# facebookresearch/dmc-net

Hardware: AMD Instinct MI355X
Metric: clips/sec (3-seg 224x224) DMC-gen+ResNet-18 train step (higher is better)
Workload: dtype f32

## Files before the change

### dmc-net_amd/csrc/conv_x3s.hip

```cpp
#include "dmc_common.h"
#include "x3s_common.h"
#include <type_traits>

using namespace dmc;
using namespace dmc::x3;

namespace {

__global__ __launch_bounds__(256) void x3s_split_kernel(const float* __restrict__ x, unsigned short* __restrict__ xs, long M, int C) {
    const int c8 = C >> 3;
    const long total = M * c8;
    const int nchunk = C >> 4;
    for (long o = (long)blockIdx.x * 256 + threadIdx.x; o < total; o += (long)gridDim.x * 256) {
        const long m = o / c8;
        const int g = (int)(o - m * c8);
        const float4 a = reinterpret_cast<const float4*>(x)[2 * o], b = reinterpret_cast<const float4*>(x)[2 * o + 1];
        const float v[8] = {a.x, a.y, a.z, a.w, b.x, b.y, b.z, b.w};
        x3s_store8(xs, v, (size_t)M, nchunk, (size_t)m, g);
    }
}

__global__ __launch_bounds__(256) void x3s_merge_kernel(const unsigned short* __restrict__ xs, float* __restrict__ x, long M, int C) {
    const long total = M * C;
    const size_t plane = (size_t)M * 16;
    const int nchunk = C >> 4;
    for (long o = (long)blockIdx.x * 256 + threadIdx.x; o < total; o += (long)gridDim.x * 256) {
        const long m = o / C;
        const int c = (int)(o - m * C);
        const size_t w = ((size_t)(c >> 4) * M + m) * 16 + (c & 15);
        const float a = __uint_as_float((unsigned)xs[w] << 16);
        const float b = __uint_as_float((unsigned)xs[(size_t)nchunk * plane + w] << 16);
        const float d = __uint_as_float((unsigned)xs[(size_t)2 * nchunk * plane + w] << 16);
        x[o] = (a + b) + d;
    }
}

__global__ __launch_bounds__(256) void x3s_pack_w_kernel(const float* __restrict__ w, unsigned short* __restrict__ wf,
                                                         unsigned short* __restrict__ wt, int Cout, int Cin, int mirror) {
    const bool transposed = blockIdx.y == 1;
    unsigned short* dst = transposed ? wt : wf;
    if (!dst) return;
    const int R = transposed ? Cin : Cout, K = transposed ? Cout : Cin;
    const int nchunk = K >> 4;
    const long total = (long)R * 9 * K;
    for (long i = (long)blockIdx.x * 256 + threadIdx.x; i < total; i += (long)gridDim.x * 256) {
        long t = i;
        const int kk = (int)(t & 15); t >>= 4;
        const int rl = (int)(t & 63); t >>= 6;
        const int tap = (int)(t % 9); t /= 9;
        const int ch = (int)(t % nchunk);
        const int rt = (int)(t / nchunk);
        const int r = rt * 64 + rl, k = ch * 16 + kk;
        const float v = transposed ? w[((long)k * 9 + (mirror ? 8 - tap : tap)) * Cin + r] : w[((long)r * 9 + tap) * Cin + k];
        unsigned s0, s1, s2;
        split3_bf16(v, s0, s1, s2);
        const size_t base = ((((size_t)(rt * nchunk + ch) * 9 + tap) * 3) * 64 + rl) * 16 + (kk ^ (((rl >> 3) & 1) << 3));
        dst[base] = (unsigned short)s0;
        dst[base + 64 * 16] = (unsigned short)s1;
        dst[base + 2 * 64 * 16] = (unsigned short)s2;
    }
}

struct X3Args {
    const void* xs;
    const void* wp;
    float* y;
    const float* addend;
    double* stat_part;
    int N, H, W, K, R;
    int M;
    unsigned plane_bytes;
    const float* bnb_y = nullptr;
    const float* bnb_stats = nullptr;
    const float* bnb_gamma = nullptr;
    const float* bnb_beta = nullptr;
    const unsigned char* bnb_mask = nullptr;
    int bnb_relu = 0;
    double* bnb_part = nullptr;
    int part_blocks = -1;
    int ablate;
};
struct X3EvalArgs : X3Args {
    const float* stats;
    const float* gamma;
    const float* beta;
    const float* res;
    unsigned short* ys;
    int s2d, relu;
};

template <int WM, int WN, int TM, int TN, int PPMAX, bool STAG = false, int CLS = 1, bool EVAL = false>
__global__ __launch_bounds__(WM * WN * 64) void x3s_conv_kernel(std::conditional_t<EVAL, X3EvalArgs, X3Args> a) {
    static_assert(!EVAL || CLS == 1, "the eval epilogue belongs to the forward convolution");
    constexpr int NW = WM * WN, BM = 32 * TM * WM, BN = 32 * TN * WN;
    static_assert(BN == 64, "packed weight image is 64 rows wide");
    static_assert(PPMAX % 32 == 0 || PPMAX % 32 == 1, "patch transfers move 32 pixel rows");
    constexpr int PSL = PPMAX * 32;
    constexpr int PB = 3 * PSL;
    constexpr int WB = 3 * 3 * BN * 32;
    constexpr int WOFF = 2 * PB;
    static_assert(!STAG || NW >= 4, "two transfer groups need four waves");
    constexpr int NA = STAG ? NW / 2 : NW, NB = NW - (STAG ? NA : 0);
    constexpr int NDW = (PPMAX / 32 + NA - 1) / NA;
    constexpr int NEW = WB / 1024;
    constexpr int NEWW = (NEW + NB - 1) / NB;
    extern __shared__ __attribute__((aligned(1024))) char lds_x3[];

    const int tid = threadIdx.x, lane = tid & 63;
    const int wave = __builtin_amdgcn_readfirstlane(tid >> 6);
    const int wm = wave % WM, wn = wave / WM;
    const int l31 = lane & 31, khalf = lane >> 5;
    const unsigned lds0 = lds_addr_of(lds_x3);

    const int HW = a.H * a.W, PW = a.W;
    constexpr int ZROW = PPMAX - 1;
    const int m0 = blockIdx.x * BM;
    const int mlast = (m0 + BM < a.M ? m0 + BM : a.M) - 1;
    const int r_first = m0 / PW, r_last = mlast / PW;
    const int f0 = (r_first > 0 ? r_first - 1 : 0) * PW;
    const int f1 = (r_last + 2) * PW < a.M ? (r_last + 2) * PW : a.M;
    const int PP = f1 - f0;
    const int ND = (PP + 31) >> 5;

    unsigned pvoff[NDW];
#pragma unroll
    for (int k = 0; k < NDW; ++k) {
        const int pr = 32 * (wave + NA * k) + (lane >> 1), h = lane & 1;
        pvoff[k] = pr < PP ? (unsigned)(f0 + pr) * 32u + (unsigned)((h ^ ((pr >> 3) & 1)) << 4) : OOB;
    }
    int xaddr[TM][9];
#pragma unroll
    for (int i = 0; i < TM; ++i) {
        int m = m0 + (wm * TM + i) * 32 + l31;
        if (m > mlast) m = mlast;
        const int n = m / HW, rem = m - n * HW, yy = rem / a.W, xx = rem - yy * a.W;
        const int pp = m - f0;
#pragma unroll
        for (int t = 0; t < 9; ++t) {
            const int dx = CLS == 4 ? (t % 3 == 0 ? 1 : 0) : t % 3 - 1, dy = CLS == 4 ? (t / 3 == 0 ? 1 : 0) : t / 3 - 1;
            const int row = (xx + dx >= 0 && xx + dx < a.W && yy + dy >= 0 && yy + dy < a.H) ? pp + dy * PW + dx : ZROW;
            xaddr[i][t] = row * 32 + ((khalf ^ ((row >> 3) & 1)) << 4);
        }
    }
    const int waddr = (wn * TN * 32 + l31) * 32 + ((khalf ^ ((l31 >> 3) & 1)) << 4);

    const u32x4 srd_x = make_srd(a.xs);
    const int nchunk = a.K >> 4, S = 3 * nchunk;
    const u32x4 srd_w = make_srd(reinterpret_cast<const char*>(a.wp) + (size_t)blockIdx.y * S * WB);
    const unsigned lane16 = (unsigned)lane * 16u;

    const bool grp_a = wave < NA, grp_b = !STAG || wave >= NA;
    const int wb = STAG ? wave - NA : wave;
    auto dma_weight = [&](int step, int wbuf, int k) {
        const int e = wb + NB * k;
        if (e < NEW) dma_buf16(srd_w, lane16, (unsigned)(step * WB + e * 1024), lds0 + WOFF + wbuf * WB + e * 1024);
    };
    auto dma_patch = [&](int chunk, int slice, int pbuf, int k) {
        const int d = wave + NA * k;
        if (d < ND) dma_buf16(srd_x, pvoff[k], (unsigned)(slice * nchunk + chunk) * a.plane_bytes, lds0 + pbuf * PB + slice * PSL + d * 1024);
    };
    auto issue_weights = [&](int step, int wbuf) {
        if (grp_b) {
#pragma unroll
            for (int k = 0; k < NEWW; ++k) dma_weight(step, wbuf, k);
        }
    };
    auto issue_patch = [&](int chunk, int slice, int pbuf) {
        if (grp_a) {
#pragma unroll
            for (int k = 0; k < NDW; ++k) dma_patch(chunk, slice, pbuf, k);
        }
    };

    f32x16 acc[CLS][TM][TN];
#pragma unroll
    for (int cl = 0; cl < CLS; ++cl)
#pragma unroll
        for (int i = 0; i < TM; ++i)
#pragma unroll
            for (int j = 0; j < TN; ++j)
#pragma unroll
                for (int e = 0; e < 16; ++e) acc[cl][i][j][e] = 0.f;

    lds_cptr const L = (lds_cptr)lds_x3;
    struct Frag { u32x4 X[TM][3], W[TN][3]; };
    auto load_frags = [&](auto pbufc, auto wbufc, auto tc, Frag& f) {
        constexpr int pbuf = decltype(pbufc)::value, wbuf = decltype(wbufc)::value, t = decltype(tc)::value;
#pragma unroll
        for (int s = 0; s < 3; ++s) {
#pragma unroll
            for (int j = 0; j < TN; ++j)
                f.W[j][s] = *reinterpret_cast<const __attribute__((address_space(3))) u32x4*>(
                    L + waddr + (WOFF + wbuf * WB + (((t % 3) * 3 + s) * BN + 32 * j) * 32));
#pragma unroll
            for (int i = 0; i < TM; ++i)
                f.X[i][s] = *reinterpret_cast<const __attribute__((address_space(3))) u32x4*>(L + xaddr[i][t] + (pbuf * PB + s * PSL));
        }
    };
    auto mfma_frags = [&](const Frag& f, auto tc, auto&& between) {
        constexpr int t = decltype(tc)::value;
        constexpr int cl = CLS == 4 ? (t / 3 != 1) * 2 + (t % 3 != 1) : 0;
#pragma unroll
        for (int p = 0; p < 6; ++p) {
            constexpr int WS[6] = {0, 0, 0, 1, 1, 2}, XS[6] = {2, 1, 0, 1, 0, 0};
#pragma unroll
            for (int i = 0; i < TM; ++i)
#pragma unroll
                for (int j = 0; j < TN; ++j) acc[cl][i][j] = mfma_bf16(f.W[j][WS[p]], f.X[i][XS[p]], acc[cl][i][j]);
            between(p);
        }
    };
    auto nothing = [](int) {};
    constexpr int NRD = 3 * (TM + TN), NMF = 6 * TM * TN;
    auto interleave = [&]() {
#pragma unroll
        for (int k = 0; k < NRD; ++k) {
            __builtin_amdgcn_sched_group_barrier(0x008, 1, 0);
            __builtin_amdgcn_sched_group_barrier(0x100, 1, 0);
        }
        __builtin_amdgcn_sched_group_barrier(0x008, NMF - NRD, 0);
    };
    const bool dma_on = !(DMC_ABL(a.ablate) & 64);
    auto step = [&](auto pbufc, auto wbufc, auto qc, Frag& FA, Frag& FB, int c) {
        constexpr int pbuf = decltype(pbufc)::value, wbuf = decltype(wbufc)::value, q = decltype(qc)::value;
        using NP = std::integral_constant<int, q == 2 ? (pbuf ^ 1) : pbuf>;
        using NWB = std::integral_constant<int, wbuf ^ 1>;
        using NT = std::integral_constant<int, q == 2 ? 0 : 3 * (q + 1)>;
        using T0 = std::integral_constant<int, 3 * q>;
        using T1 = std::integral_constant<int, 3 * q + 1>;
        using T2 = std::integral_constant<int, 3 * q + 2>;
        const int s = 3 * c + q;
        load_frags(pbufc, wbufc, std::integral_constant<int, 3 * q + 1>{}, FB);
        if constexpr (STAG) {
            const bool go = grp_b && dma_on && s + 1 < S;
            mfma_frags(FA, T0{}, [&](int p) {
                if (go) {
#pragma unroll
                    for (int k = p; k < NEWW; k += 6) dma_weight(s + 1, wbuf ^ 1, k);
                }
            });
        } else {
            mfma_frags(FA, T0{}, nothing);
            interleave();
        }
        load_frags(pbufc, wbufc, std::integral_constant<int, 3 * q + 2>{}, FA);
        mfma_frags(FB, T1{}, nothing);
        interleave();
        if (DMC_ABL(a.ablate) & 16) asm volatile("s_waitcnt lgkmcnt(0)" ::: "memory");
        else asm volatile("s_waitcnt vmcnt(0) lgkmcnt(0)" ::: "memory");
        __builtin_amdgcn_s_barrier();
        const int vc = q == 2 ? c + 2 : c + 1;
        if constexpr (STAG) {
            if (s + 1 < S) load_frags(NP{}, NWB{}, NT{}, FB);
            const bool go = grp_a && dma_on && vc < nchunk;
            mfma_frags(FA, T2{}, [&](int p) {
                if (go) {
#pragma unroll
                    for (int k = p; k < NDW; k += 6) dma_patch(vc, q == 2 ? 0 : q + 1, q == 2 ? pbuf : (pbuf ^ 1), k);
                }
            });
        } else {
            if (dma_on) {
                if (s + 2 < S) issue_weights(s + 2, wbuf);
                if (vc < nchunk) issue_patch(vc, q == 2 ? 0 : q + 1, q == 2 ? pbuf : (pbuf ^ 1));
            }
            if (s + 1 < S) load_frags(NP{}, NWB{}, NT{}, FB);
            mfma_frags(FA, T2{}, nothing);
        }
    };
    using I0 = std::integral_constant<int, 0>;
    using I1 = std::integral_constant<int, 1>;
    using Q0 = std::integral_constant<int, 0>;
    using Q1 = std::integral_constant<int, 1>;
    using Q2 = std::integral_constant<int, 2>;

    if (tid < 12)
        *reinterpret_cast<float4*>(lds_x3 + (tid >> 1) * PSL + ZROW * 32 + (tid & 1) * 16) = make_float4(0.f, 0.f, 0.f, 0.f);
    issue_weights(0, 0);
    issue_patch(0, 0, 0); issue_patch(0, 1, 0); issue_patch(0, 2, 0);
    asm volatile("s_waitcnt vmcnt(0)" ::: "memory");
    __builtin_amdgcn_s_barrier();
    if (dma_on) {
        if (!STAG && S > 1) issue_weights(1, 1);
        if (nchunk > 1) issue_patch(1, 0, 1);
    }
    Frag F0, F1;
    load_frags(I0{}, I0{}, Q0{}, F0);
#pragma unroll 1
    for (int c = 0; c < ((DMC_ABL(a.ablate) & 256) ? 0 : nchunk); c += 2) {
        step(I0{}, I0{}, Q0{}, F0, F1, c);
        step(I0{}, I1{}, Q1{}, F1, F0, c);
        step(I0{}, I0{}, Q2{}, F0, F1, c);
        step(I1{}, I1{}, Q0{}, F1, F0, c + 1);
        step(I1{}, I0{}, Q1{}, F0, F1, c + 1);
        step(I1{}, I1{}, Q2{}, F1, F0, c + 1);
    }

    static_assert(WN == 1 && TN == 2, "epilogue: a wave owns all 64 channels of its pixels");
    constexpr int EP = 272, ETILE = 32 * TM * EP;
    char* etile = lds_x3 + wave * ETILE;
    const int mw0 = m0 + wm * TM * 32;
    const int rbase = blockIdx.y * BN;
#pragma unroll
    for (int cl = 0; cl < CLS; ++cl) {
#pragma unroll
        for (int i = 0; i < TM; ++i) {
            const bool ok = mw0 + 32 * i + l31 <= mlast;
#pragma unroll
            for (int j = 0; j < TN; ++j)
#pragma unroll
                for (int g = 0; g < 4; ++g) {
                    float4 v = make_float4(acc[cl][i][j][4 * g], acc[cl][i][j][4 * g + 1], acc[cl][i][j][4 * g + 2], acc[cl][i][j][4 * g + 3]);
                    if (!ok) v = make_float4(0.f, 0.f, 0.f, 0.f);
                    *reinterpret_cast<float4*>(etile + (32 * i + l31) * EP + (32 * j + 8 * g + 4 * khalf) * 4) = v;
                }
        }
        if constexpr (EVAL) {
            const int c4 = rbase + (lane & 15) * 4;
            const float4 mean = *reinterpret_cast<const float4*>(a.stats + c4), istd = *reinterpret_cast<const float4*>(a.stats + a.R + c4);
            const float4 gm = *reinterpret_cast<const float4*>(a.gamma + c4), bt = *reinterpret_cast<const float4*>(a.beta + c4);
            const bool has_res = a.res != nullptr, relu = a.relu != 0;
            const int ochunk = a.R >> 4;
#pragma unroll
            for (int it = 0; it < 8 * TM; ++it) {
                const int prow = 4 * it + (lane >> 4);
                const int m = mw0 + prow;
                const float4 v = *reinterpret_cast<const float4*>(etile + prow * EP + (lane & 15) * 16);
                if (m <= mlast) {
                    const size_t o = (size_t)m * a.R + c4;
                    float4 rv = make_float4(0.f, 0.f, 0.f, 0.f);
                    if (has_res) rv = *reinterpret_cast<const float4*>(a.res + o);
                    const float w[4] = {bn_apply_act1(v.x, mean.x, istd.x, gm.x, bt.x, has_res, rv.x, relu),
                                        bn_apply_act1(v.y, mean.y, istd.y, gm.y, bt.y, has_res, rv.y, relu),
                                        bn_apply_act1(v.z, mean.z, istd.z, gm.z, bt.z, has_res, rv.z, relu),
                                        bn_apply_act1(v.w, mean.w, istd.w, gm.w, bt.w, has_res, rv.w, relu)};
                    if (a.y) *reinterpret_cast<float4*>(a.y + o) = make_float4(w[0], w[1], w[2], w[3]);
                    if (a.ys) {
                        if (a.s2d) {
                            const int n = m / HW, rem = m - n * HW, yy = rem / a.W, xx = rem - yy * a.W;
                            const int cls = (yy & 1) * 2 + (xx & 1);
                            const size_t mq = ((size_t)n * (a.H >> 1) + (yy >> 1)) * (a.W >> 1) + (xx >> 1);
                            x3s_store4(a.ys, w, (size_t)a.M >> 2, 4 * ochunk, mq, (c4 >> 2) + cls * 4 * ochunk);
                        } else {
                            x3s_store4(a.ys, w, (size_t)a.M, ochunk, (size_t)m, c4 >> 2);
                        }
                    }
                }
            }
        } else
        if (!(DMC_ABL(a.ablate) & 128)) {
#pragma unroll
            for (int it = 0; it < 8 * TM; ++it) {
                const int prow = 4 * it + (lane >> 4);
                const int m = mw0 + prow;
                float4 v = *reinterpret_cast<const float4*>(etile + prow * EP + (lane & 15) * 16);
                if (m <= mlast) {
                    size_t opix = (size_t)m;
                    if (CLS == 4) {
                        const int n = m / HW, rem = m - n * HW, ya = rem / a.W, xb = rem - ya * a.W;
                        opix = ((size_t)n * (2 * a.H) + 2 * ya + (cl >> 1)) * (2 * a.W) + 2 * xb + (cl & 1);
                    }
                    const size_t o = opix * a.R + rbase + (lane & 15) * 4;
                    if (a.addend) {
                        const float4 av = *reinterpret_cast<const float4*>(a.addend + o);
                        v.x += av.x; v.y += av.y; v.z += av.z; v.w += av.w;
                    }
                    *reinterpret_cast<float4*>(a.y + o) = v;
                    if (CLS == 1 && a.bnb_part) {
                        const int c4 = rbase + (lane & 15) * 4;
                        const float4 yv = *reinterpret_cast<const float4*>(a.bnb_y + o);
                        const float4 mean = *reinterpret_cast<const float4*>(a.bnb_stats + c4);
                        const float4 istd = *reinterpret_cast<const float4*>(a.bnb_stats + a.R + c4);
                        const float4 xh = make_float4((yv.x - mean.x) * istd.x, (yv.y - mean.y) * istd.y, (yv.z - mean.z) * istd.z, (yv.w - mean.w) * istd.w);
                        if (a.bnb_relu) {
                            unsigned mb;
                            if (a.bnb_mask) {
                                mb = a.bnb_mask[o >> 2];
                            } else {
                                const float4 g = *reinterpret_cast<const float4*>(a.bnb_gamma + c4), b = *reinterpret_cast<const float4*>(a.bnb_beta + c4);
                                mb = (fmaf(xh.x, g.x, b.x) > 0.f ? 1u : 0u) | (fmaf(xh.y, g.y, b.y) > 0.f ? 2u : 0u) |
                                     (fmaf(xh.z, g.z, b.z) > 0.f ? 4u : 0u) | (fmaf(xh.w, g.w, b.w) > 0.f ? 8u : 0u);
                            }
                            v.x = (mb & 1) ? v.x : 0.f; v.y = (mb & 2) ? v.y : 0.f; v.z = (mb & 4) ? v.z : 0.f; v.w = (mb & 8) ? v.w : 0.f;
                        }
                        *reinterpret_cast<float4*>(etile + prow * EP + (lane & 15) * 16) = v;
                        *reinterpret_cast<float4*>(etile + NW * ETILE + 8192 + prow * EP + (lane & 15) * 16) = xh;
                    }
                } else if (CLS == 1 && a.bnb_part) {
                    *reinterpret_cast<float4*>(etile + prow * EP + (lane & 15) * 16) = make_float4(0.f, 0.f, 0.f, 0.f);
                    *reinterpret_cast<float4*>(etile + NW * ETILE + 8192 + prow * EP + (lane & 15) * 16) = make_float4(0.f, 0.f, 0.f, 0.f);
                }
            }
        }
    }
    if constexpr (EVAL) return;
    if (CLS == 1 && a.bnb_part) {
        double* red = reinterpret_cast<double*>(lds_x3 + NW * ETILE);
        const char* xtile = etile + NW * ETILE + 8192;
        double d1 = 0.0, d2 = 0.0;
#pragma unroll 8
        for (int p = 0; p < 32 * TM; ++p) {
            const double d = (double)*reinterpret_cast<const float*>(etile + p * EP + lane * 4);
            const double xh = (double)*reinterpret_cast<const float*>(xtile + p * EP + lane * 4);
            d1 += d;
            d2 += d * xh;
        }
        red[(wm * 64 + lane) * 2 + 0] = d1;
        red[(wm * 64 + lane) * 2 + 1] = d2;
        __syncthreads();
        for (int cc = tid; cc < BN; cc += NW * 64) {
            double e1 = 0.0, e2 = 0.0;
#pragma unroll
            for (int w = 0; w < WM; ++w) { e1 += red[(w * 64 + cc) * 2 + 0]; e2 += red[(w * 64 + cc) * 2 + 1]; }
            double* dst = a.bnb_part + ((size_t)blockIdx.x * a.R + rbase + cc) * 2;
            dst[0] = e1; dst[1] = e2;
        }
    }
    if (CLS == 1 && a.stat_part) {
        double* red = reinterpret_cast<double*>(lds_x3 + NW * ETILE);
        double d1 = 0.0, d2 = 0.0;
#pragma unroll 8
        for (int p = 0; p < 32 * TM; ++p) {
            const double v = (double)*reinterpret_cast<const float*>(etile + p * EP + lane * 4);
            d1 += v;
            d2 += v * v;
        }
        red[(wm * 64 + lane) * 2 + 0] = d1;
        red[(wm * 64 + lane) * 2 + 1] = d2;
        __syncthreads();
        for (int c = tid; c < BN; c += NW * 64) {
            double e1 = 0.0, e2 = 0.0;
#pragma unroll
            for (int w = 0; w < WM; ++w) { e1 += red[(w * 64 + c) * 2 + 0]; e2 += red[(w * 64 + c) * 2 + 1]; }
            double* dst = a.stat_part + ((size_t)blockIdx.x * a.R + rbase + c) * 2;
            dst[0] = e1; dst[1] = e2;
        }
    }
}

int patch_pixels_max(int N, int H, int W, int BM) {
    const long M = (long)N * H * W;
    int worst = 0;
    long tiles = (M + BM - 1) / BM;
    if (tiles > W) tiles = W;
    for (long t = 0; t < tiles; ++t) {
        const long m0 = t * BM, ml = (m0 + BM < M ? m0 + BM : M) - 1;
        const long r0 = m0 / W, r1 = ml / W;
        const long f0 = (r0 > 0 ? r0 - 1 : 0) * W, f1 = (r1 + 2) * W;
        if ((int)(f1 - f0) + 1 > worst) worst = (int)(f1 - f0) + 1;
    }
    return worst;
}

struct X3Cfg { int id, BM, PPMAX, threads; };
constexpr X3Cfg X3CFGS[] = {{0, 256, 608, 512}, {1, 128, 320, 256}, {2, 64, 192, 128}, {3, 256, 608, 256}, {4, 128, 225, 256}};

bool x3s_shape_ok(int N, int H, int W, int K, int R) {
    if (N <= 0 || H <= 0 || W <= 0 || K % 32 != 0 || R % 64 != 0 || K <= 0 || R <= 0) return false;
    const long M = (long)N * H * W;
    return M * (K > R ? K : R) * 6 < (1L << 31);
}

int x3s_choose(int N, int H, int W, int R) {
    const long M = (long)N * H * W;
    const int forced = option(OPT_CONV_CFG);
    if (forced >= 101 && forced <= 105 && patch_pixels_max(N, H, W, X3CFGS[forced - 101].BM) <= X3CFGS[forced - 101].PPMAX) return forced - 101;
    if (forced != 106 && patch_pixels_max(N, H, W, X3CFGS[4].BM) <= X3CFGS[4].PPMAX && ((M + X3CFGS[4].BM - 1) / X3CFGS[4].BM) * (R / 64) >= 512)
        return 4;
    int fallback = -1;
    for (const X3Cfg& c : X3CFGS) {
        if (c.id > 2 || patch_pixels_max(N, H, W, c.BM) > c.PPMAX) continue;
        const long wgs = ((M + c.BM - 1) / c.BM) * (R / 64);
        if (wgs >= 160) return c.id;
        fallback = c.id;
    }
    return fallback;
}

template <int WM, int TM, int PPMAX>
int launch_x3s(const X3Args& a, hipStream_t s) {
    constexpr int BM = 32 * TM * WM;
    constexpr size_t op_bytes = 2 * 3 * PPMAX * 32 + 2 * 3 * 3 * 64 * 32, ep_bytes = 2 * (size_t)BM * 272 + 8192;
    constexpr size_t lds_bytes = op_bytes > ep_bytes ? op_bytes : ep_bytes;
    dim3 grid((a.M + BM - 1) / BM, a.R / 64);
    if ((a.stat_part || a.bnb_part) && a.part_blocks >= 0 && (unsigned)a.part_blocks != grid.x)
        return fail(DMC_E_INVALID, "x3s_conv: statistics partials have %d rows but this launch writes %u (dmc_x3s_conv_stat_blocks was "
                                   "called under another conv_cfg option?)", a.part_blocks, grid.x);
    if constexpr (WM >= 4) {
        if (!(option(OPT_CONV_ABLATE) & 512)) {
            static LdsLimit lim_attr2;
    const hipError_t attr2 = lim_attr2.raise(reinterpret_cast<const void*>(&x3s_conv_kernel<WM, 1, TM, 2, PPMAX, true>), (int)lds_bytes);
            if (attr2 != hipSuccess) return fail(DMC_E_LAUNCH, "x3s_conv: cannot raise the dynamic LDS limit: %s", hipGetErrorString(attr2));
            x3s_conv_kernel<WM, 1, TM, 2, PPMAX, true><<<grid, WM * 64, lds_bytes, s>>>(a);
            return check_launch("x3s_conv");
        }
    }
    static LdsLimit lim_attr;
    const hipError_t attr = lim_attr.raise(reinterpret_cast<const void*>(&x3s_conv_kernel<WM, 1, TM, 2, PPMAX>), (int)lds_bytes);
    if (attr != hipSuccess) return fail(DMC_E_LAUNCH, "x3s_conv: cannot raise the dynamic LDS limit: %s", hipGetErrorString(attr));
    x3s_conv_kernel<WM, 1, TM, 2, PPMAX><<<grid, WM * 64, lds_bytes, s>>>(a);
    return check_launch("x3s_conv");
}

struct X3Bnb { const float *y, *stats, *gamma, *beta; const unsigned char* mask; int relu; double* part; };

int run_x3s(const void* xs, const void* wp, const float* addend, float* y, double* stat_part, int part_blocks, int N, int H, int W,
            int K, int R, hipStream_t s, const X3Bnb* bnb = nullptr) {
    if (!xs || !wp || !y) return fail(DMC_E_INVALID, "x3s_conv: null pointer");
    if (!x3s_shape_ok(N, H, W, K, R)) return fail(DMC_E_INVALID, "x3s_conv: unsupported shape N=%d H=%d W=%d K=%d R=%d", N, H, W, K, R);
    const int cfg = x3s_choose(N, H, W, R);
    X3Args a;
    a.xs = xs; a.wp = wp; a.y = y; a.addend = addend; a.stat_part = stat_part;
    a.N = N; a.H = H; a.W = W; a.K = K; a.R = R; a.M = N * H * W;
    a.plane_bytes = (unsigned)a.M * 32u;
    a.part_blocks = part_blocks;
    if ((stat_part || bnb) && part_blocks <= 0) return fail(DMC_E_INVALID, "x3s_conv: stat_blocks must be the row count of the partials");
    if (bnb) {
        a.bnb_y = bnb->y; a.bnb_stats = bnb->stats; a.bnb_gamma = bnb->gamma; a.bnb_beta = bnb->beta; a.bnb_mask = bnb->mask;
        a.bnb_relu = bnb->relu; a.bnb_part = bnb->part;
    }
    a.ablate = option(OPT_CONV_ABLATE);
    if (DMC_ABL(a.ablate) & 32) a.stat_part = nullptr;
    switch (cfg) {
        case 0: return launch_x3s<8, 1, 608>(a, s);
        case 1: return launch_x3s<4, 1, 320>(a, s);
        case 2: return launch_x3s<2, 1, 192>(a, s);
        case 3: return launch_x3s<4, 2, 608>(a, s);
        case 4: return launch_x3s<4, 1, 225>(a, s);
        default: return fail(DMC_E_INVALID, "x3s_conv: the patch of a %d x %d image does not fit the LDS", H, W);
    }
}

template <int WM, int TM, int PPMAX>
int launch_x3s_eval(const X3EvalArgs& a, hipStream_t s) {
    constexpr int BM = 32 * TM * WM;
    constexpr size_t lds_bytes = 2 * 3 * PPMAX * 32 + 2 * 3 * 3 * 64 * 32;
    static_assert((size_t)BM * 272 <= lds_bytes, "the epilogue tiles live in the operand LDS");
    dim3 grid((a.M + BM - 1) / BM, a.R / 64);
    static LdsLimit lim_attr;
    const hipError_t attr = lim_attr.raise(reinterpret_cast<const void*>(&x3s_conv_kernel<WM, 1, TM, 2, PPMAX, (WM >= 4), 1, true>), (int)lds_bytes);
    if (attr != hipSuccess) return fail(DMC_E_LAUNCH, "x3s_conv_bn_eval: cannot raise the dynamic LDS limit: %s", hipGetErrorString(attr));
    x3s_conv_kernel<WM, 1, TM, 2, PPMAX, (WM >= 4), 1, true><<<grid, WM * 64, lds_bytes, s>>>(a);
    return check_launch("x3s_conv_bn_eval");
}

struct X3WgArgs {
    const void* xs;
    const void* dys;
    float* part;
    int N, H, Cin, Cout;
    unsigned plane_bytes;
    int steps, per_group, tiles_ci;
};

template <int W_, int R>
struct WgGeom {
    static constexpr int PW = W_ + 2;
    static constexpr int NGRP = R >= W_ + 2 ? 2 : 4, LA = NGRP / 2;
    static constexpr int NRING = NGRP * R;
    static constexpr int XPX = NRING * PW;
    static constexpr int XPL = ((XPX + 3) / 8) * 8 + 4;
    static constexpr int NPX = R * W_;
    static constexpr int NKB = (NPX + 15) / 16;
    static constexpr int DYP = NKB * 16;
    static constexpr int DYT = ((DYP + 31) / 32) * 32;
    static constexpr int DYPL = ((DYT + 3) / 8) * 8 + 4;
    static constexpr int XI = (R * PW + 31) / 32;
    static constexpr int DI = DYT / 32;
    static constexpr int XBYTES = 12 * XPL * 32, DYBYTES = 12 * DYPL * 32;
    static constexpr int LDS = XBYTES + 2 * DYBYTES;
};

template <int W_, int R>
__global__ __launch_bounds__(768) void x3s_wgrad_kernel(X3WgArgs a) {
    using G = WgGeom<W_, R>;
    constexpr int PW = G::PW, NRING = G::NRING, XPL = G::XPL, DYPL = G::DYPL, NKB = G::NKB;
    extern __shared__ __attribute__((aligned(1024))) char lds_wg[];
    const int tid = threadIdx.x, lane = tid & 63;
    const int wave = __builtin_amdgcn_readfirstlane(tid >> 6);
    const int l31 = lane & 31, khalf = lane >> 5, L = lane & 15, grp = (lane >> 4) & 1;
    const int quarter = wave & 3, trow = wave >> 2;
    const int wi = quarter & 1, wj = quarter >> 1;
    const int tci = blockIdx.x % a.tiles_ci, tco = blockIdx.x / a.tiles_ci;
    const unsigned lds0 = lds_addr_of(lds_wg);
    const int HP = a.H + 2;
    const int s_begin = blockIdx.y * a.per_group;
    const int s_end = s_begin + a.per_group < a.steps ? s_begin + a.per_group : a.steps;
    const u32x4 srd_x = make_srd(a.xs), srd_d = make_srd(a.dys);
    const unsigned soff_x = (unsigned)((wave >> 2) * (a.Cin >> 4) + tci * 4 + (wave & 3)) * a.plane_bytes;
    const unsigned soff_d = (unsigned)((wave >> 2) * (a.Cout >> 4) + tco * 4 + (wave & 3)) * a.plane_bytes;
    const unsigned xplane = lds0 + (unsigned)wave * XPL * 32, dplane = lds0 + G::XBYTES + (unsigned)wave * DYPL * 32;
    const int lpx = lane >> 1;
    const unsigned lhalf = (unsigned)(lane & 1) << 4;

    const unsigned img_bytes = (unsigned)(a.H * W_) * 32u;
    unsigned xpre[G::XI], dpre[G::DI];
#pragma unroll
    for (int i = 0; i < G::XI; ++i) {
        const int px = 32 * i + lpx;
        const int r = px / PW, col = px - r * PW - 1;
        xpre[i] = (col >= 0 && col < W_) ? (unsigned)(r * W_ + col) * 32u + lhalf : NOPIX;
    }
#pragma unroll
    for (int i = 0; i < G::DI; ++i) {
        const int p = 32 * i + lpx;
        dpre[i] = p < G::NPX ? (unsigned)p * 32u + lhalf : NOPIX;
    }
    auto issue_x = [&](int q, const WgGroupPos& g) {
        const int slot0 = (((q % G::NGRP) + G::NGRP) % G::NGRP) * R;
        unsigned tbase, img_off;
        wg_group_base(g, a.N, W_, img_bytes, tbase, img_off);
#pragma unroll
        for (int i = 0; i < G::XI; ++i)
            if (32 * i + lpx < R * PW)
                dma_buf16(srd_x, wg_lane_off(tbase, xpre[i], img_bytes), soff_x + img_off, xplane + (unsigned)(slot0 * PW + 32 * i) * 32u);
    };
    auto issue_dy = [&](const WgGroupPos& g, int buf) {
        unsigned tbase, img_off;
        wg_group_base(g, a.N, W_, img_bytes, tbase, img_off);
#pragma unroll
        for (int i = 0; i < G::DI; ++i)
            dma_buf16(srd_d, wg_lane_off(tbase, dpre[i], img_bytes), soff_d + img_off, dplane + (unsigned)buf * G::DYBYTES + (unsigned)(32 * i) * 32u);
    };

    f32x16 acc[3];
// ... 89 lines not shown
    p.per_group = (p.steps + groups - 1) / groups;
    p.groups = (p.steps + p.per_group - 1) / p.per_group;
    return true;
}

template <int W_, int R>
int launch_x3s_wgrad(const X3WgPlan& p, X3WgArgs a, float* dw, hipStream_t s) {
    using G = WgGeom<W_, R>;
    static_assert(G::LDS <= 160 * 1024, "weight-gradient tiles exceed the LDS");
    static LdsLimit lim_attr;
    const hipError_t attr = lim_attr.raise(reinterpret_cast<const void*>(&x3s_wgrad_kernel<W_, R>), G::LDS);
    if (attr != hipSuccess) return fail(DMC_E_LAUNCH, "x3s_wgrad: cannot raise the dynamic LDS limit: %s", hipGetErrorString(attr));
    x3s_wgrad_kernel<W_, R><<<dim3(p.tiles, p.groups), 768, G::LDS, s>>>(a);
    int rc = check_launch("x3s_wgrad");
    if (rc || p.groups == 1) return rc;
    const long numel = (long)a.Cout * 9 * a.Cin;
    const long blocks = (numel + 63) / 64;
    x3s_wgrad_reduce_kernel<<<(int)(blocks > 4096 ? 4096 : blocks), 256, 0, s>>>(a.part, dw, p.groups, numel);
    return check_launch("x3s_wgrad_reduce");
}

__global__ __launch_bounds__(256) void x3s_bnb_final_kernel(const double* __restrict__ part, int nblk, int C,
                                                            float* __restrict__ dgamma, float* __restrict__ dbeta) {
    __shared__ double red[2][4];
    const int c = blockIdx.x, lane = threadIdx.x & 63, wave = threadIdx.x >> 6;
    double s = 0.0, ss = 0.0;
    for (int b = threadIdx.x; b < nblk; b += 256) {
        const double2 v = *reinterpret_cast<const double2*>(part + ((size_t)b * C + c) * 2);
        s += v.x;
        ss += v.y;
    }
#pragma unroll
    for (int o = 32; o > 0; o >>= 1) { s += __shfl_down(s, o, 64); ss += __shfl_down(ss, o, 64); }
    if (lane == 0) { red[0][wave] = s; red[1][wave] = ss; }
    __syncthreads();
    if (threadIdx.x != 0) return;
    dbeta[c] = (float)(red[0][0] + red[0][1] + red[0][2] + red[0][3]);
    dgamma[c] = (float)(red[1][0] + red[1][1] + red[1][2] + red[1][3]);
}

int stream_blocks(long total) {
    long b = (total + 255) / 256;
    return (int)(b < 1 ? 1 : (b > 8192 ? 8192 : b));
}

}

extern "C" {

size_t dmc_x3s_slices_bytes(long M, int C) { return (size_t)M * (size_t)C * 6; }

int dmc_x3s_split(const float* x, void* xs, long M, int C, dmc_stream_t stream) {
    if (!x || !xs || M <= 0 || C <= 0 || C % 16 != 0) return fail(DMC_E_INVALID, "dmc_x3s_split: bad argument");
    x3s_split_kernel<<<stream_blocks(M * (C / 8)), 256, 0, (hipStream_t)stream>>>(x, static_cast<unsigned short*>(xs), M, C);
    return check_launch("x3s_split");
}

int dmc_x3s_merge(const void* xs, float* x, long M, int C, dmc_stream_t stream) {
    if (!x || !xs || M <= 0 || C <= 0 || C % 16 != 0) return fail(DMC_E_INVALID, "dmc_x3s_merge: bad argument");
    x3s_merge_kernel<<<stream_blocks(M * C), 256, 0, (hipStream_t)stream>>>(static_cast<const unsigned short*>(xs), x, M, C);
    return check_launch("x3s_merge");
}

size_t dmc_x3s_wpack_bytes(int Cin, int Cout) { return (size_t)Cin * (size_t)Cout * 9 * 6; }

int dmc_x3s_pack_weights(const float* w, void* wpack_f, void* wpack_t, int Cin, int Cout, dmc_stream_t stream) {
    if (!w || (!wpack_f && !wpack_t) || Cin % 64 != 0 || Cout % 64 != 0 || Cin <= 0 || Cout <= 0)
        return fail(DMC_E_INVALID, "dmc_x3s_pack_weights: bad argument");
    const long total = (long)Cin * Cout * 9;
    x3s_pack_w_kernel<<<dim3(stream_blocks(total) > 1024 ? 1024 : stream_blocks(total), 2), 256, 0, (hipStream_t)stream>>>(
        w, static_cast<unsigned short*>(wpack_f), static_cast<unsigned short*>(wpack_t), Cout, Cin, 1);
    return check_launch("x3s_pack_w");
}

int dmc_x3s_conv_supported(int N, int H, int W, int Cin, int Cout) {
    return Cin % 64 == 0 && Cout % 64 == 0 && x3s_shape_ok(N, H, W, Cin, Cout) && x3s_shape_ok(N, H, W, Cout, Cin) &&
           x3s_choose(N, H, W, Cout) >= 0 && x3s_choose(N, H, W, Cin) >= 0 ? 1 : 0;
}

int dmc_x3s_conv_stat_blocks(int N, int H, int W, int Cout) {
    const int cfg = x3s_choose(N, H, W, Cout);
    if (cfg < 0) return 0;
    const long M = (long)N * H * W;
    return (int)((M + X3CFGS[cfg].BM - 1) / X3CFGS[cfg].BM);
}

int dmc_x3s_conv_fwd(const void* xs, const void* wpack_f, float* y, double* stat_partials, int stat_blocks, int N, int H, int W,
                     int Cin, int Cout, dmc_stream_t stream) {
    return run_x3s(xs, wpack_f, nullptr, y, stat_partials, stat_blocks, N, H, W, Cin, Cout, (hipStream_t)stream);
}

int dmc_x3s_conv_bn_eval(const void* xs, const void* wpack_f, const float* stats, const float* gamma, const float* beta,
                         const float* residual, float* y, void* ys, int s2d, int relu, int N, int H, int W, int Cin, int Cout,
                         dmc_stream_t stream) {
    if (!xs || !wpack_f || !stats || !gamma || !beta) return fail(DMC_E_INVALID, "dmc_x3s_conv_bn_eval: null pointer");
    if (!y && !ys) return fail(DMC_E_INVALID, "dmc_x3s_conv_bn_eval: no output (y and ys are both null)");
    if (s2d && !ys) return fail(DMC_E_INVALID, "dmc_x3s_conv_bn_eval: s2d describes the slice output, which is null");
    if (s2d && ((H & 1) || (W & 1))) return fail(DMC_E_INVALID, "dmc_x3s_conv_bn_eval: a space-to-depth result needs even H and W (H=%d W=%d)", H, W);
    if (Cin % 64 != 0 || Cout % 64 != 0 || !x3s_shape_ok(N, H, W, Cin, Cout) || !x3s_shape_ok(N, H, W, Cout, Cin))
        return fail(DMC_E_INVALID, "dmc_x3s_conv_bn_eval: unsupported shape N=%d H=%d W=%d Cin=%d Cout=%d", N, H, W, Cin, Cout);
    X3EvalArgs a;
    a.xs = xs; a.wp = wpack_f; a.y = y; a.addend = nullptr; a.stat_part = nullptr;
    a.N = N; a.H = H; a.W = W; a.K = Cin; a.R = Cout; a.M = N * H * W;
    a.plane_bytes = (unsigned)a.M * 32u;
    a.ablate = 0;
    a.stats = stats; a.gamma = gamma; a.beta = beta; a.res = residual; a.ys = static_cast<unsigned short*>(ys);
    a.s2d = s2d ? 1 : 0; a.relu = relu ? 1 : 0;
    hipStream_t s = (hipStream_t)stream;
    switch (x3s_choose(N, H, W, Cout)) {
        case 0: return launch_x3s_eval<8, 1, 608>(a, s);
        case 1: return launch_x3s_eval<4, 1, 320>(a, s);
        case 2: return launch_x3s_eval<2, 1, 192>(a, s);
        case 3: return launch_x3s_eval<4, 2, 608>(a, s);
        case 4: return launch_x3s_eval<4, 1, 225>(a, s);
        default: return fail(DMC_E_INVALID, "dmc_x3s_conv_bn_eval: the patch of a %d x %d image does not fit the LDS", H, W);
    }
}

int dmc_x3s_conv_dgrad(const void* dys, const void* wpack_t, const float* addend, float* dx, int N, int H, int W, int Cin, int Cout,
                       dmc_stream_t stream) {
    return run_x3s(dys, wpack_t, addend, dx, nullptr, -1, N, H, W, Cout, Cin, (hipStream_t)stream);
}

int dmc_x3s_conv_wgrad_supported(int N, int H, int W, int Cin, int Cout) {
    X3WgPlan p;
    return x3s_wgrad_plan(N, H, W, Cin, Cout, p) && x3s_shape_ok(N, H, W, Cin, Cout) && x3s_shape_ok(N, H, W, Cout, Cin) ? 1 : 0;
}

size_t dmc_x3s_conv_wgrad_bytes(int N, int H, int W, int Cin, int Cout) {
    X3WgPlan p;
    if (!x3s_wgrad_plan(N, H, W, Cin, Cout, p) || p.groups <= 1) return 0;
    return (size_t)p.groups * Cout * 9 * Cin * sizeof(float);
}

int dmc_x3s_conv_wgrad(const void* xs, const void* dys, float* dw, float* workspace, int N, int H, int W, int Cin, int Cout,
                       dmc_stream_t stream) {
    X3WgPlan p;
    if (!xs || !dys || !dw) return fail(DMC_E_INVALID, "dmc_x3s_conv_wgrad: null pointer");
    if (!dmc_x3s_conv_wgrad_supported(N, H, W, Cin, Cout) || !x3s_wgrad_plan(N, H, W, Cin, Cout, p))
        return fail(DMC_E_INVALID, "dmc_x3s_conv_wgrad: unsupported shape N=%d H=%d W=%d Cin=%d Cout=%d", N, H, W, Cin, Cout);
    if (p.groups > 1 && !workspace) return fail(DMC_E_INVALID, "dmc_x3s_conv_wgrad: workspace required");
    X3WgArgs a;
    a.xs = xs; a.dys = dys; a.part = p.groups > 1 ? workspace : dw;
    a.N = N; a.H = H; a.Cin = Cin; a.Cout = Cout;
    a.plane_bytes = (unsigned)((long)N * H * W) * 32u;
    a.steps = p.steps; a.per_group = p.per_group; a.tiles_ci = Cin / 64;
    hipStream_t s = (hipStream_t)stream;
    switch (W) {
        case 56: return launch_x3s_wgrad<56, 1>(p, a, dw, s);
        case 28: return launch_x3s_wgrad<28, 2>(p, a, dw, s);
        case 14: return launch_x3s_wgrad<14, 4>(p, a, dw, s);
        default: return launch_x3s_wgrad<7, 9>(p, a, dw, s);
    }
}

int dmc_x3s_conv_dgrad_s2_supported(int N, int OH, int OW, int Cin, int Cout) {
    return Cin % 64 == 0 && Cout % 64 == 0 && x3s_shape_ok(N, OH, OW, Cout, Cin) && (long)N * OH * OW * 4 * Cin * 4 < (1L << 40) &&
           patch_pixels_max(N, OH, OW, 128) <= 320 ? 1 : 0;
}

int dmc_x3s_pack_weights_s2(const float* w, void* wpack_t2, int Cin, int Cout, dmc_stream_t stream) {
    if (!w || !wpack_t2 || Cin % 64 != 0 || Cout % 64 != 0 || Cin <= 0 || Cout <= 0)
        return fail(DMC_E_INVALID, "dmc_x3s_pack_weights_s2: bad argument");
    const long total = (long)Cin * Cout * 9;
    x3s_pack_w_kernel<<<dim3(stream_blocks(total) > 1024 ? 1024 : stream_blocks(total), 2), 256, 0, (hipStream_t)stream>>>(
        w, nullptr, static_cast<unsigned short*>(wpack_t2), Cout, Cin, 0);
    return check_launch("x3s_pack_w_s2");
}

int dmc_x3s_conv_dgrad_s2(const void* dys, const void* wpack_t2, float* dx, int N, int OH, int OW, int Cin, int Cout,
                          dmc_stream_t stream) {
    if (!dys || !wpack_t2 || !dx) return fail(DMC_E_INVALID, "dmc_x3s_conv_dgrad_s2: null pointer");
    if (!dmc_x3s_conv_dgrad_s2_supported(N, OH, OW, Cin, Cout))
        return fail(DMC_E_INVALID, "dmc_x3s_conv_dgrad_s2: unsupported shape N=%d OH=%d OW=%d Cin=%d Cout=%d", N, OH, OW, Cin, Cout);
    X3Args a;
    a.xs = dys; a.wp = wpack_t2; a.y = dx; a.addend = nullptr; a.stat_part = nullptr;
    a.N = N; a.H = OH; a.W = OW; a.K = Cout; a.R = Cin; a.M = N * OH * OW;
    a.plane_bytes = (unsigned)a.M * 32u;
    a.ablate = option(OPT_CONV_ABLATE);
    constexpr size_t lds_bytes = 2 * 3 * 320 * 32 + 2 * 3 * 3 * 64 * 32;
    static LdsLimit lim_attr;
    const hipError_t attr = lim_attr.raise(reinterpret_cast<const void*>(&x3s_conv_kernel<4, 1, 1, 2, 320, true, 4>), (int)lds_bytes);
    if (attr != hipSuccess) return fail(DMC_E_LAUNCH, "x3s_conv_dgrad_s2: cannot raise the dynamic LDS limit: %s", hipGetErrorString(attr));
    dim3 grid((a.M + 127) / 128, Cin / 64);
    x3s_conv_kernel<4, 1, 1, 2, 320, true, 4><<<grid, 256, lds_bytes, (hipStream_t)stream>>>(a);
    return check_launch("x3s_conv_dgrad_s2");
}

int dmc_x3s_conv_dgrad_bnb(const void* dys, const void* wpack_t, const float* addend, float* dx, const float* bn_y,
                           const float* bn_stats, const float* bn_gamma, const float* bn_beta, const unsigned char* bn_relu_mask,
                           int bn_relu, double* partials, int stat_blocks, float* dgamma, float* dbeta, int N, int H, int W, int Cin,
                           int Cout, dmc_stream_t stream) {
    if (!bn_y || !bn_stats || !bn_gamma || !bn_beta || !partials || !dgamma || !dbeta)
        return fail(DMC_E_INVALID, "dmc_x3s_conv_dgrad_bnb: null pointer");
    X3Bnb b = {bn_y, bn_stats, bn_gamma, bn_beta, bn_relu_mask, bn_relu, partials};
    int rc = run_x3s(dys, wpack_t, addend, dx, nullptr, stat_blocks, N, H, W, Cout, Cin, (hipStream_t)stream, &b);
    if (rc) return rc;
    x3s_bnb_final_kernel<<<Cin, 256, 0, (hipStream_t)stream>>>(partials, stat_blocks, Cin, dgamma, dbeta);
    return check_launch("x3s_bnb_final");
}

}
```

Before: 3542.

## Add row-aligned 512-pixel conv tiles for 56-wide maps with fused BN-backward epilogue

Result: faster. 3596 (median of 6 runs) (+1.5%).

```diff
diff --git a/dmc-net_amd/csrc/conv_x3s.hip b/dmc-net_amd/csrc/conv_x3s.hip
--- a/dmc-net_amd/csrc/conv_x3s.hip
+++ b/dmc-net_amd/csrc/conv_x3s.hip
@@ -79,6 +79,7 @@
     double* bnb_part = nullptr;
     int part_blocks = -1;
     int ablate;
+    int bms = 0;
 };
 struct X3EvalArgs : X3Args {
     const float* stats;
@@ -89,9 +90,10 @@
     int s2d, relu;
 };
 
-template <int WM, int WN, int TM, int TN, int PPMAX, bool STAG = false, int CLS = 1, bool EVAL = false>
+template <int WM, int WN, int TM, int TN, int PPMAX, bool STAG = false, int CLS = 1, bool EVAL = false, bool ROWT = false>
 __global__ __launch_bounds__(WM * WN * 64) void x3s_conv_kernel(std::conditional_t<EVAL, X3EvalArgs, X3Args> a) {
     static_assert(!EVAL || CLS == 1, "the eval epilogue belongs to the forward convolution");
+    static_assert(!ROWT || CLS == 1, "row-aligned tiles: forward and stride-1 data gradient");
     constexpr int NW = WM * WN, BM = 32 * TM * WM, BN = 32 * TN * WN;
     static_assert(BN == 64, "packed weight image is 64 rows wide");
     static_assert(PPMAX % 32 == 0 || PPMAX % 32 == 1, "patch transfers move 32 pixel rows");
@@ -114,8 +116,9 @@
 
     const int HW = a.H * a.W, PW = a.W;
     constexpr int ZROW = PPMAX - 1;
-    const int m0 = blockIdx.x * BM;
-    const int mlast = (m0 + BM < a.M ? m0 + BM : a.M) - 1;
+    const int bms = ROWT ? a.bms : BM;
+    const int m0 = blockIdx.x * bms;
+    const int mlast = (m0 + bms < a.M ? m0 + bms : a.M) - 1;
     const int r_first = m0 / PW, r_last = mlast / PW;
     const int f0 = (r_first > 0 ? r_first - 1 : 0) * PW;
     const int f1 = (r_last + 2) * PW < a.M ? (r_last + 2) * PW : a.M;
@@ -186,6 +189,12 @@
     struct Frag { u32x4 X[TM][3], W[TN][3]; };
     auto load_frags = [&](auto pbufc, auto wbufc, auto tc, Frag& f) {
         constexpr int pbuf = decltype(pbufc)::value, wbuf = decltype(wbufc)::value, t = decltype(tc)::value;
+        int xa[TM];
+#pragma unroll
+        for (int i = 0; i < TM; ++i) {
+            xa[i] = xaddr[i][t];
+            if constexpr (ROWT && pbuf == 1) asm volatile("" : "+v"(xa[i]));
+        }
 #pragma unroll
         for (int s = 0; s < 3; ++s) {
 #pragma unroll
@@ -194,7 +203,7 @@
                     L + waddr + (WOFF + wbuf * WB + (((t % 3) * 3 + s) * BN + 32 * j) * 32));
 #pragma unroll
             for (int i = 0; i < TM; ++i)
-                f.X[i][s] = *reinterpret_cast<const __attribute__((address_space(3))) u32x4*>(L + xaddr[i][t] + (pbuf * PB + s * PSL));
+                f.X[i][s] = *reinterpret_cast<const __attribute__((address_space(3))) u32x4*>(L + xa[i] + (pbuf * PB + s * PSL));
         }
     };
     auto mfma_frags = [&](const Frag& f, auto tc, auto&& between) {
@@ -301,6 +310,78 @@
     char* etile = lds_x3 + wave * ETILE;
     const int mw0 = m0 + wm * TM * 32;
     const int rbase = blockIdx.y * BN;
+    if constexpr (ROWT && !EVAL) {
+        if (a.bnb_part) {
+            constexpr int ET1 = 32 * EP;
+            char* dtile = lds_x3 + wave * 2 * ET1;
+            char* xtile = dtile + ET1;
+            const int c4 = rbase + (lane & 15) * 4;
+            const float4 mean = *reinterpret_cast<const float4*>(a.bnb_stats + c4);
+            const float4 istd = *reinterpret_cast<const float4*>(a.bnb_stats + a.R + c4);
+            double d1 = 0.0, d2 = 0.0;
+#pragma unroll
+            for (int i = 0; i < TM; ++i) {
+                const bool ok = mw0 + 32 * i + l31 <= mlast;
+#pragma unroll
+                for (int j = 0; j < TN; ++j)
+#pragma unroll
+                    for (int g = 0; g < 4; ++g) {
+                        float4 v = make_float4(acc[0][i][j][4 * g], acc[0][i][j][4 * g + 1], acc[0][i][j][4 * g + 2], acc[0][i][j][4 * g + 3]);
+                        if (!ok) v = make_float4(0.f, 0.f, 0.f, 0.f);
+                        *reinterpret_cast<float4*>(dtile + l31 * EP + (32 * j + 8 * g + 4 * khalf) * 4) = v;
+                    }
+#pragma unroll
+                for (int it = 0; it < 8; ++it) {
+                    const int prow = 4 * it + (lane >> 4);
+                    const int m = mw0 + 32 * i + prow;
+                    float4 v = *reinterpret_cast<const float4*>(dtile + prow * EP + (lane & 15) * 16);
+                    float4 xh = make_float4(0.f, 0.f, 0.f, 0.f);
+                    if (m <= mlast) {
+                        const size_t o = (size_t)m * a.R + c4;
+                        if (a.addend) {
+                            const float4 av = *reinterpret_cast<const float4*>(a.addend + o);
+                            v.x += av.x; v.y += av.y; v.z += av.z; v.w += av.w;
+                        }
+                        *reinterpret_cast<float4*>(a.y + o) = v;
+                        const float4 yv = *reinterpret_cast<const float4*>(a.bnb_y + o);
+                        xh = make_float4((yv.x - mean.x) * istd.x, (yv.y - mean.y) * istd.y, (yv.z - mean.z) * istd.z, (yv.w - mean.w) * istd.w);
+                        if (a.bnb_relu) {
+                            unsigned mb;
+                            if (a.bnb_mask) {
+                                mb = a.bnb_mask[o >> 2];
+                            } else {
+                                const float4 g = *reinterpret_cast<const float4*>(a.bnb_gamma + c4), b = *reinterpret_cast<const float4*>(a.bnb_beta + c4);
+                                mb = (fmaf(xh.x, g.x, b.x) > 0.f ? 1u : 0u) | (fmaf(xh.y, g.y, b.y) > 0.f ? 2u : 0u) |
+                                     (fmaf(xh.z, g.z, b.z) > 0.f ? 4u : 0u) | (fmaf(xh.w, g.w, b.w) > 0.f ? 8u : 0u);
+                            }
+                            v.x = (mb & 1) ? v.x : 0.f; v.y = (mb & 2) ? v.y : 0.f; v.z = (mb & 4) ? v.z : 0.f; v.w = (mb & 8) ? v.w : 0.f;
+                        }
+                    }
+                    *reinterpret_cast<float4*>(dtile + prow * EP + (lane & 15) * 16) = v;
+                    *reinterpret_cast<float4*>(xtile + prow * EP + (lane & 15) * 16) = xh;
+                }
+#pragma unroll 8
+                for (int p = 0; p < 32; ++p) {
+                    const double d = (double)*reinterpret_cast<const float*>(dtile + p * EP + lane * 4);
+                    const double xh = (double)*reinterpret_cast<const float*>(xtile + p * EP + lane * 4);
+                    d1 += d;
+                    d2 += d * xh;
+                }
+            }
+            double* red = reinterpret_cast<double*>(lds_x3 + NW * 2 * ET1);
+            red[(wm * 64 + lane) * 2 + 0] = d1;
+            red[(wm * 64 + lane) * 2 + 1] = d2;
+            __syncthreads();
+            for (int cc = tid; cc < BN; cc += NW * 64) {
+                double e1 = 0.0, e2 = 0.0;
+#pragma unroll
+                for (int w = 0; w < WM; ++w) { e1 += red[(w * 64 + cc) * 2 + 0]; e2 += red[(w * 64 + cc) * 2 + 1]; }
+                double* dst = a.bnb_part + ((size_t)blockIdx.x * a.R + rbase + cc) * 2;
+                dst[0] = e1; dst[1] = e2;
+            }
+            return;
+        }
+    }
 #pragma unroll
     for (int cl = 0; cl < CLS; ++cl) {
 #pragma unroll
@@ -453,7 +534,14 @@
 }
 
 struct X3Cfg { int id, BM, PPMAX, threads; };
-constexpr X3Cfg X3CFGS[] = {{0, 256, 608, 512}, {1, 128, 320, 256}, {2, 64, 192, 128}, {3, 256, 608, 256}, {4, 128, 225, 256}};
+constexpr X3Cfg X3CFGS[] = {{0, 256, 608, 512}, {1, 128, 320, 256}, {2, 64, 192, 128}, {3, 256, 608, 256}, {4, 128, 225, 256},
+                            {5, 512, 640, 512}};
+
+int x3s_tile_stride(int cfg, int W) { return cfg == 5 ? (W <= X3CFGS[5].BM ? (X3CFGS[5].BM / W) * W : 0) : X3CFGS[cfg].BM; }
+bool x3s_row_tiles_fit(int W) {
+    const int stride = x3s_tile_stride(5, W);
+    return stride > 0 && stride + 2 * W + 1 <= X3CFGS[5].PPMAX;
+}
 
 bool x3s_shape_ok(int N, int H, int W, int K, int R) {
     if (N <= 0 || H <= 0 || W <= 0 || K % 32 != 0 || R % 64 != 0 || K <= 0 || R <= 0) return false;
@@ -465,8 +553,14 @@
     const long M = (long)N * H * W;
     const int forced = option(OPT_CONV_CFG);
     if (forced >= 101 && forced <= 105 && patch_pixels_max(N, H, W, X3CFGS[forced - 101].BM) <= X3CFGS[forced - 101].PPMAX) return forced - 101;
+    if (forced == 107 && x3s_row_tiles_fit(W)) return 5;
     if (forced != 106 && patch_pixels_max(N, H, W, X3CFGS[4].BM) <= X3CFGS[4].PPMAX && ((M + X3CFGS[4].BM - 1) / X3CFGS[4].BM) * (R / 64) >= 512)
         return 4;
+    if (forced != 108 && W == 56 && x3s_row_tiles_fit(W) && patch_pixels_max(N, H, W, X3CFGS[0].BM) <= X3CFGS[0].PPMAX) {
+        const long r5 = (((M + x3s_tile_stride(5, W) - 1) / x3s_tile_stride(5, W)) * (R / 64) + 255) / 256;
+        const long r0 = (((M + X3CFGS[0].BM - 1) / X3CFGS[0].BM) * (R / 64) + 255) / 256;
+        if (9 * r5 < 5 * r0) return 5;
+    }
     int fallback = -1;
     for (const X3Cfg& c : X3CFGS) {
         if (c.id > 2 || patch_pixels_max(N, H, W, c.BM) > c.PPMAX) continue;
@@ -477,28 +571,31 @@
     return fallback;
 }
 
-template <int WM, int TM, int PPMAX>
+template <int WM, int TM, int PPMAX, bool ROWT = false>
 int launch_x3s(const X3Args& a, hipStream_t s) {
     constexpr int BM = 32 * TM * WM;
-    constexpr size_t op_bytes = 2 * 3 * PPMAX * 32 + 2 * 3 * 3 * 64 * 32, ep_bytes = 2 * (size_t)BM * 272 + 8192;
+    constexpr size_t op_bytes = 2 * 3 * PPMAX * 32 + 2 * 3 * 3 * 64 * 32, ep_bytes = (ROWT ? 1 : 2) * (size_t)BM * 272 + 8192;
     constexpr size_t lds_bytes = op_bytes > ep_bytes ? op_bytes : ep_bytes;
-    dim3 grid((a.M + BM - 1) / BM, a.R / 64);
+    static_assert(lds_bytes <= 160 * 1024 && (!ROWT || 2 * WM * 32 * 272 + 8192 <= lds_bytes), "the tiles exceed the LDS");
+    dim3 grid((a.M + a.bms - 1) / a.bms, a.R / 64);
     if ((a.stat_part || a.bnb_part) && a.part_blocks >= 0 && (unsigned)a.part_blocks != grid.x)
         return fail(DMC_E_INVALID, "x3s_conv: statistics partials have %d rows but this launch writes %u (dmc_x3s_conv_stat_blocks was "
                                    "called under another conv_cfg option?)", a.part_blocks, grid.x);
     if constexpr (WM >= 4) {
-        if (!(option(OPT_CONV_ABLATE) & 512)) {
+        if (ROWT || !(option(OPT_CONV_ABLATE) & 512)) {
             static LdsLimit lim_attr2;
-    const hipError_t attr2 = lim_attr2.raise(reinterpret_cast<const void*>(&x3s_conv_kernel<WM, 1, TM, 2, PPMAX, true>), (int)lds_bytes);
+    const hipError_t attr2 = lim_attr2.raise(reinterpret_cast<const void*>(&x3s_conv_kernel<WM, 1, TM, 2, PPMAX, true, 1, false, ROWT>), (int)lds_bytes);
             if (attr2 != hipSuccess) return fail(DMC_E_LAUNCH, "x3s_conv: cannot raise the dynamic LDS limit: %s", hipGetErrorString(attr2));
-            x3s_conv_kernel<WM, 1, TM, 2, PPMAX, true><<<grid, WM * 64, lds_bytes, s>>>(a);
+            x3s_conv_kernel<WM, 1, TM, 2, PPMAX, true, 1, false, ROWT><<<grid, WM * 64, lds_bytes, s>>>(a);
             return check_launch("x3s_conv");
         }
     }
-    static LdsLimit lim_attr;
-    const hipError_t attr = lim_attr.raise(reinterpret_cast<const void*>(&x3s_conv_kernel<WM, 1, TM, 2, PPMAX>), (int)lds_bytes);
-    if (attr != hipSuccess) return fail(DMC_E_LAUNCH, "x3s_conv: cannot raise the dynamic LDS limit: %s", hipGetErrorString(attr));
-    x3s_conv_kernel<WM, 1, TM, 2, PPMAX><<<grid, WM * 64, lds_bytes, s>>>(a);
+    if constexpr (!ROWT) {
+        static LdsLimit lim_attr;
+        const hipError_t attr = lim_attr.raise(reinterpret_cast<const void*>(&x3s_conv_kernel<WM, 1, TM, 2, PPMAX>), (int)lds_bytes);
+        if (attr != hipSuccess) return fail(DMC_E_LAUNCH, "x3s_conv: cannot raise the dynamic LDS limit: %s", hipGetErrorString(attr));
+        x3s_conv_kernel<WM, 1, TM, 2, PPMAX><<<grid, WM * 64, lds_bytes, s>>>(a);
+    }
     return check_launch("x3s_conv");
 }
 
@@ -514,6 +611,7 @@
     a.N = N; a.H = H; a.W = W; a.K = K; a.R = R; a.M = N * H * W;
     a.plane_bytes = (unsigned)a.M * 32u;
     a.part_blocks = part_blocks;
+    a.bms = cfg >= 0 ? x3s_tile_stride(cfg, W) : 0;
     if ((stat_part || bnb) && part_blocks <= 0) return fail(DMC_E_INVALID, "x3s_conv: stat_blocks must be the row count of the partials");
     if (bnb) {
         a.bnb_y = bnb->y; a.bnb_stats = bnb->stats; a.bnb_gamma = bnb->gamma; a.bnb_beta = bnb->beta; a.bnb_mask = bnb->mask;
@@ -527,20 +625,21 @@
         case 2: return launch_x3s<2, 1, 192>(a, s);
         case 3: return launch_x3s<4, 2, 608>(a, s);
         case 4: return launch_x3s<4, 1, 225>(a, s);
+        case 5: return launch_x3s<8, 2, 640, true>(a, s);
         default: return fail(DMC_E_INVALID, "x3s_conv: the patch of a %d x %d image does not fit the LDS", H, W);
     }
 }
 
-template <int WM, int TM, int PPMAX>
+template <int WM, int TM, int PPMAX, bool ROWT = false>
 int launch_x3s_eval(const X3EvalArgs& a, hipStream_t s) {
     constexpr int BM = 32 * TM * WM;
     constexpr size_t lds_bytes = 2 * 3 * PPMAX * 32 + 2 * 3 * 3 * 64 * 32;
-    static_assert((size_t)BM * 272 <= lds_bytes, "the epilogue tiles live in the operand LDS");
-    dim3 grid((a.M + BM - 1) / BM, a.R / 64);
+    static_assert((size_t)BM * 272 <= lds_bytes && lds_bytes <= 160 * 1024, "the epilogue tiles live in the operand LDS");
+    dim3 grid((a.M + a.bms - 1) / a.bms, a.R / 64);
     static LdsLimit lim_attr;
-    const hipError_t attr = lim_attr.raise(reinterpret_cast<const void*>(&x3s_conv_kernel<WM, 1, TM, 2, PPMAX, (WM >= 4), 1, true>), (int)lds_bytes);
+    const hipError_t attr = lim_attr.raise(reinterpret_cast<const void*>(&x3s_conv_kernel<WM, 1, TM, 2, PPMAX, (WM >= 4), 1, true, ROWT>), (int)lds_bytes);
     if (attr != hipSuccess) return fail(DMC_E_LAUNCH, "x3s_conv_bn_eval: cannot raise the dynamic LDS limit: %s", hipGetErrorString(attr));
-    x3s_conv_kernel<WM, 1, TM, 2, PPMAX, (WM >= 4), 1, true><<<grid, WM * 64, lds_bytes, s>>>(a);
+    x3s_conv_kernel<WM, 1, TM, 2, PPMAX, (WM >= 4), 1, true, ROWT><<<grid, WM * 64, lds_bytes, s>>>(a);
     return check_launch("x3s_conv_bn_eval");
 }
 
@@ -796,7 +895,8 @@
     const int cfg = x3s_choose(N, H, W, Cout);
     if (cfg < 0) return 0;
     const long M = (long)N * H * W;
-    return (int)((M + X3CFGS[cfg].BM - 1) / X3CFGS[cfg].BM);
+    const int stride = x3s_tile_stride(cfg, W);
+    return (int)((M + stride - 1) / stride);
 }
 
 int dmc_x3s_conv_fwd(const void* xs, const void* wpack_f, float* y, double* stat_partials, int stat_blocks, int N, int H, int W,
@@ -821,12 +921,15 @@
     a.stats = stats; a.gamma = gamma; a.beta = beta; a.res = residual; a.ys = static_cast<unsigned short*>(ys);
     a.s2d = s2d ? 1 : 0; a.relu = relu ? 1 : 0;
     hipStream_t s = (hipStream_t)stream;
-    switch (x3s_choose(N, H, W, Cout)) {
+    const int cfg = x3s_choose(N, H, W, Cout);
+    a.bms = cfg >= 0 ? x3s_tile_stride(cfg, W) : 0;
+    switch (cfg) {
         case 0: return launch_x3s_eval<8, 1, 608>(a, s);
         case 1: return launch_x3s_eval<4, 1, 320>(a, s);
         case 2: return launch_x3s_eval<2, 1, 192>(a, s);
         case 3: return launch_x3s_eval<4, 2, 608>(a, s);
         case 4: return launch_x3s_eval<4, 1, 225>(a, s);
+        case 5: return launch_x3s_eval<8, 2, 640, true>(a, s);
         default: return fail(DMC_E_INVALID, "dmc_x3s_conv_bn_eval: the patch of a %d x %d image does not fit the LDS", H, W);
     }
 }
@@ -892,6 +995,7 @@
     a.N = N; a.H = OH; a.W = OW; a.K = Cout; a.R = Cin; a.M = N * OH * OW;
     a.plane_bytes = (unsigned)a.M * 32u;
     a.ablate = option(OPT_CONV_ABLATE);
+    a.bms = 128;
     constexpr size_t lds_bytes = 2 * 3 * 320 * 32 + 2 * 3 * 3 * 64 * 32;
     static LdsLimit lim_attr;
     const hipError_t attr = lim_attr.raise(reinterpret_cast<const void*>(&x3s_conv_kernel<4, 1, 1, 2, 320, true, 4>), (int)lds_bytes);
```
